# tschnz/Live-Video-Magnification

Measured on AMD Instinct MI355X. Metric: magnified frames/sec at 1080p, Laplace-motion 6 levels; % HBM roofline, higher is better.
Workload: dtype f32

## Files before the change

include/lvm_hip.h:

```cpp
#ifndef LVM_HIP_H
#define LVM_HIP_H
#include <stddef.h>
#include <stdint.h>
#ifdef __cplusplus
extern "C" {
#endif

enum lvm_mode { LVM_MODE_LAPLACE = 0, LVM_MODE_PHASE = 1, LVM_MODE_COLOR = 2, LVM_MODE_NONE = 3 };

enum lvm_status {
    LVM_OK = 0,
    LVM_ERR_INVALID = -1,
    LVM_ERR_HIP = -2,
    LVM_ERR_NO_DEVICE = -3,
    LVM_ERR_OOM = -4
};

typedef struct lvm_params {
    int32_t  mode;
    int32_t  levels;
    double   amplification;
    double   coWavelength;
    double   coLow;
    double   coHigh;
// ... 131 lines not shown
                       ptrdiff_t* chroma_stride);
int  lvm_canvas_convert_device(lvm_ctx* ctx, int fmt, const uint8_t* d_bgr, int w, int h, ptrdiff_t bgr_stride, ptrdiff_t bgr_frame_stride, int n_frames,
                               uint8_t* d_out, ptrdiff_t out_stride, ptrdiff_t out_frame_stride, void* hip_stream);

int  lvm_set_pipeline(lvm_ctx* ctx, int depth);
int  lvm_flush(lvm_ctx* ctx, void* hip_stream);

int  lvm_synchronize(lvm_ctx* ctx);

const char* lvm_last_error(lvm_ctx* ctx);

int  lvm_max_levels(int w, int h);
int  lvm_optimal_buffer_size(int fps);
void lvm_butterworth2(double Wn, double a[3], double b[3]);

int  lvm_debug_keep_float(lvm_ctx* ctx, int on);
int  lvm_debug_read_float(lvm_ctx* ctx, float* dst, size_t count);
int  lvm_debug_exact_lab(lvm_ctx* ctx, int on);
int  lvm_debug_clock_probe_start(lvm_ctx* ctx, double max_seconds);
int  lvm_debug_clock_probe_stop(lvm_ctx* ctx, double* mhz, double* seconds);
int  lvm_debug_sweep_u8_steps(lvm_ctx* ctx, uint32_t first_bits, uint64_t count, uint64_t* mismatches, uint32_t* first_bad_bits);
int  lvm_debug_lab_analytic(lvm_ctx* ctx, int on);
int  lvm_debug_trig_eval(lvm_ctx* ctx, int fn, const float* d_x, float* d_y, size_t n, void* stream);
#define LVM_LAB_LUT_ENTRIES (33 * 33 * 33 * 3)
int  lvm_get_lab_lut(lvm_ctx* ctx, int16_t* dst);
int  lvm_set_lab_lut(lvm_ctx* ctx, const int16_t* src);
int  lvm_profile_enable(lvm_ctx* ctx, int on);
int  lvm_profile_collect(lvm_ctx* ctx);
int  lvm_profile_only(lvm_ctx* ctx, const char* name);
int  lvm_profile_entry(lvm_ctx* ctx, int idx, char* name, size_t name_cap, double* total_ms,
                       long long* launches);
int  lvm_profile_variants(lvm_ctx* ctx, int idx, char* variants, size_t cap);
double lvm_algorithmic_bytes(int mode, int w, int h, int channels, int levels, double framerate);

#ifdef __cplusplus
}
#endif
#endif
```

live-video-magnification_amd/binding.py:

```python
import ctypes as C
import dataclasses
import enum
import os
import struct

import numpy as np

_HERE = os.path.dirname(os.path.abspath(__file__))
LIB_PATH = os.environ.get("LVM_HIP_LIB") or os.path.join(_HERE, "liblvm_hip.so")


class MagnificationMode(enum.IntEnum):
    Laplace = 0
    Phase = 1
    Color = 2
    None_ = 3


@dataclasses.dataclass
class MagnificationParams:
    mode: int = MagnificationMode.Laplace
    amplification: float = 0.0
    coWavelength: float = 0.0
    coLow: float = 0.0
# ... 43 lines not shown


class LvmOverlayLabel(C.Structure):
    _fields_ = [("x", C.c_int32), ("y", C.c_int32), ("w", C.c_int32), ("h", C.c_int32), ("n_classes", C.c_int32),
                ("cls", C.c_void_p), ("fn", C.c_void_p)]


class LvmPreprocessParams(C.Structure):
    _fields_ = [("downscale", C.c_int32), ("roi_enabled", C.c_int32), ("roiX", C.c_float), ("roiY", C.c_float),
                ("roiW", C.c_float), ("roiH", C.c_float), ("grayscale", C.c_int32)]


def to_c_preprocess(pre, grayscale=False):
    return LvmPreprocessParams(int(pre.downscale), 1 if pre.roiEnabled else 0, pre.roiX, pre.roiY, pre.roiW, pre.roiH,
                               1 if grayscale else 0)


class LvmError(RuntimeError):
    pass


SYMBOLS = ["lvm_create", "lvm_destroy", "lvm_reset", "lvm_process", "lvm_process_device", "lvm_process_device_frames", "lvm_set_pipeline", "lvm_flush", "lvm_synchronize",
           "lvm_last_error", "lvm_max_levels", "lvm_optimal_buffer_size", "lvm_butterworth2",
           "lvm_debug_keep_float", "lvm_debug_read_float", "lvm_debug_exact_lab", "lvm_debug_sweep_u8_steps", "lvm_debug_clock_probe_start", "lvm_debug_clock_probe_stop", "lvm_debug_lab_analytic", "lvm_debug_trig_eval", "lvm_get_lab_lut", "lvm_set_lab_lut", "lvm_profile_enable", "lvm_profile_collect", "lvm_profile_only",
           "lvm_profile_entry", "lvm_profile_variants", "lvm_algorithmic_bytes", "lvm_export_geometry", "lvm_export_frames", "lvm_export_set_overlay", "lvm_overlay_device", "lvm_tile_riesz_stage1", "lvm_tile_riesz_planes", "lvm_tile_riesz_stage2",
           "lvm_preprocess_geometry", "lvm_preprocess_device", "lvm_chain_process", "lvm_chain_process_batch",
           "lvm_set_max_frames", "lvm_host_alloc", "lvm_host_free", "lvm_compose_geometry", "lvm_compose_device", "lvm_chain_process_batch_ex",
           "lvm_chain_present", "lvm_mjpeg_bound", "lvm_mjpeg_encode_device", "lvm_export_frames_mjpeg", "lvm_mjpeg_decode_device", "lvm_export_mjpeg_frames", "lvm_mjpeg_set_restart_interval", "lvm_mjpeg_set_decoder", "lvm_mjpeg_set_samplings",
           "lvm_set_opencv_build", "lvm_get_opencv_build", "lvm_set_phase_on_gray", "lvm_get_phase_on_gray",
           "lvm_set_source_format", "lvm_get_source_format",
           "lvm_set_canvas_format", "lvm_get_canvas_format", "lvm_canvas_layout", "lvm_canvas_convert_device"]


def bind(lib):
    vp = C.c_void_p
    lib.lvm_create.argtypes = [C.c_int, C.c_int, C.POINTER(vp)]
    lib.lvm_destroy.argtypes = [vp]
    lib.lvm_destroy.restype = None
    lib.lvm_reset.argtypes = [vp]
    lib.lvm_process.argtypes = [vp, C.POINTER(LvmParams), vp, C.c_int, C.c_int, C.c_int, C.c_ssize_t,
                                vp, C.c_ssize_t, C.POINTER(C.c_int)]
    lib.lvm_process_device.argtypes = [vp, C.POINTER(LvmParams), vp, C.c_int, C.c_int, C.c_int, C.c_ssize_t,
                                       C.c_ssize_t, vp, C.c_ssize_t, C.c_ssize_t, C.POINTER(C.c_int), vp]
    lib.lvm_synchronize.argtypes = [vp]
    lib.lvm_process_device_frames.argtypes = [vp, C.POINTER(LvmParams), C.c_int, vp, C.c_int, C.c_int, C.c_int, C.c_ssize_t,
                                              C.c_ssize_t, C.c_ssize_t, vp, C.c_ssize_t, C.c_ssize_t, C.c_ssize_t,
                                              C.POINTER(C.c_int), vp]
    lib.lvm_set_pipeline.argtypes = [vp, C.c_int]
    lib.lvm_flush.argtypes = [vp, vp]
    lib.lvm_last_error.argtypes = [vp]
    lib.lvm_last_error.restype = C.c_char_p
    lib.lvm_max_levels.argtypes = [C.c_int, C.c_int]
    lib.lvm_optimal_buffer_size.argtypes = [C.c_int]
    lib.lvm_butterworth2.argtypes = [C.c_double, C.POINTER(C.c_double), C.POINTER(C.c_double)]
    lib.lvm_butterworth2.restype = None
    lib.lvm_debug_keep_float.argtypes = [vp, C.c_int]
    lib.lvm_debug_read_float.argtypes = [vp, vp, C.c_size_t]
    lib.lvm_debug_exact_lab.argtypes = [vp, C.c_int]
    lib.lvm_debug_lab_analytic.argtypes = [vp, C.c_int]
    lib.lvm_debug_clock_probe_start.argtypes = [vp, C.c_double]
    lib.lvm_debug_clock_probe_stop.argtypes = [vp, C.POINTER(C.c_double), C.POINTER(C.c_double)]
    lib.lvm_debug_sweep_u8_steps.argtypes = [vp, C.c_uint32, C.c_uint64, C.POINTER(C.c_uint64), C.POINTER(C.c_uint32)]
    lib.lvm_debug_trig_eval.argtypes = [vp, C.c_int, vp, vp, C.c_size_t, vp]
    lib.lvm_get_lab_lut.argtypes = [vp, vp]
    lib.lvm_set_lab_lut.argtypes = [vp, vp]
    lib.lvm_profile_enable.argtypes = [vp, C.c_int]
    lib.lvm_profile_collect.argtypes = [vp]
    lib.lvm_profile_only.argtypes = [vp, C.c_char_p]
    lib.lvm_profile_entry.argtypes = [vp, C.c_int, C.c_char_p, C.c_size_t, C.POINTER(C.c_double),
                                      C.POINTER(C.c_longlong)]
    lib.lvm_profile_variants.argtypes = [vp, C.c_int, C.c_char_p, C.c_size_t]
    lib.lvm_algorithmic_bytes.argtypes = [C.c_int, C.c_int, C.c_int, C.c_int, C.c_int, C.c_double]
    lib.lvm_algorithmic_bytes.restype = C.c_double
    ip = C.POINTER(C.c_int)
    lib.lvm_preprocess_geometry.argtypes = [C.POINTER(LvmPreprocessParams), C.c_int, C.c_int, C.c_int, ip, ip, ip, ip, ip, ip, ip]
    lib.lvm_preprocess_device.argtypes = [vp, C.POINTER(LvmPreprocessParams), vp, C.c_int, C.c_int, C.c_int, C.c_ssize_t,
                                          C.c_ssize_t, vp, C.c_ssize_t, C.c_ssize_t, vp]
    lib.lvm_chain_process.argtypes = [vp, C.POINTER(LvmPreprocessParams), C.POINTER(LvmParams), vp, C.c_int, C.c_int, C.c_int,
                                      C.c_ssize_t, vp, C.c_ssize_t, ip]
    lib.lvm_chain_process_batch.argtypes = [vp, C.POINTER(LvmPreprocessParams), C.POINTER(LvmParams), C.POINTER(vp), C.c_int, C.c_int,
                                            C.c_int, C.c_ssize_t, C.POINTER(vp), C.c_ssize_t, ip]
    lib.lvm_chain_process_batch_ex.argtypes = [vp, C.POINTER(LvmPreprocessParams), C.POINTER(LvmParams), C.POINTER(vp), C.c_int, C.c_int,
                                               C.c_int, C.c_ssize_t, C.POINTER(vp), C.c_ssize_t, C.POINTER(vp), C.c_ssize_t, ip]
    lib.lvm_chain_present.argtypes = [vp, C.POINTER(LvmPreprocessParams), C.POINTER(LvmParams), vp, C.c_int, C.c_int, C.c_int, C.c_ssize_t,
                                      vp, C.c_ssize_t, vp, C.c_ssize_t, ip]
    lib.lvm_export_geometry.argtypes = [C.POINTER(LvmPreprocessParams), C.c_int, C.c_int, C.c_int, C.c_int, ip, ip]
# ... 378 lines not shown

    def exact_lab(self, on=True):
        self._check(self.lib.lvm_debug_exact_lab(self.h, int(on)))

    def clock_probe_start(self, max_seconds=2.0):
        self._check(self.lib.lvm_debug_clock_probe_start(self.h, float(max_seconds)))

    def clock_probe_stop(self):
        mhz, sec = C.c_double(0), C.c_double(0)
        self._check(self.lib.lvm_debug_clock_probe_stop(self.h, C.byref(mhz), C.byref(sec)))
        return float(mhz.value), float(sec.value)

    def sweep_u8_steps(self, first_bits=0, count=1 << 32):
        bad, fb = C.c_uint64(0), C.c_uint32(0)
        self._check(self.lib.lvm_debug_sweep_u8_steps(self.h, first_bits, count, C.byref(bad), C.byref(fb)))
        return int(bad.value), int(fb.value)

    def lab_analytic(self, on=True):
        self._check(self.lib.lvm_debug_lab_analytic(self.h, int(on)))

    def trig_eval(self, fn, d_x, d_y, n, stream=None):
        self._check(self.lib.lvm_debug_trig_eval(self.h, int(fn), d_x, d_y, int(n), stream))

    def lab_lut(self):
        a = np.empty(LAB_LUT_ENTRIES, np.int16)
        self._check(self.lib.lvm_get_lab_lut(self.h, a.ctypes.data))
        return a

    def set_lab_lut(self, table):
        a = np.ascontiguousarray(table, np.int16).reshape(-1)
        assert a.size == LAB_LUT_ENTRIES
        self._check(self.lib.lvm_set_lab_lut(self.h, a.ctypes.data))

    def profile(self, on=True):
        self._check(self.lib.lvm_profile_enable(self.h, int(on)))

    def profile_only(self, name=None):
        self._check(self.lib.lvm_profile_only(self.h, name.encode() if name else None))

    def profile_collect(self):
        n = self.lib.lvm_profile_collect(self.h)
        out = {}
        for i in range(max(n, 0)):
            name = C.create_string_buffer(64)
            ms = C.c_double()
            cnt = C.c_longlong()
# ... 49 lines not shown
```

live-video-magnification_amd/csrc/color.hip:

```cpp
#include <cmath>
#include <cstdlib>

#include <vector>

#include "pyramid.h"

namespace lvm {

__device__ __forceinline__ int fkey(float f) { const int b = __float_as_int(f); return b >= 0 ? b : b ^ 0x7fffffff; }
__device__ __forceinline__ float fkey_inv(int k) { return __int_as_float(k >= 0 ? k : k ^ 0x7fffffff); }

constexpr int kMMCells = 32;
struct MinMax { int mn1[kMMCells], mx1[kMMCells], mn2[kMMCells], mx2[kMMCells]; };
__device__ __forceinline__ float mm_min(const int* cells) { int k = cells[0]; for (int i = 1; i < kMMCells; ++i) k = cells[i] < k ? cells[i] : k; return fkey_inv(k); }
__device__ __forceinline__ float mm_max(const int* cells) { int k = cells[0]; for (int i = 1; i < kMMCells; ++i) k = cells[i] > k ? cells[i] : k; return fkey_inv(k); }

__device__ __forceinline__ void block_minmax(float mn, float mx, int* gmn, int* gmx) {
    __shared__ float s_mn[256], s_mx[256];
    const int t = threadIdx.x;
    s_mn[t] = mn; s_mx[t] = mx;
    __syncthreads();
    for (int s = 128; s > 0; s >>= 1) {
        if (t < s) {
            s_mn[t] = s_mn[t + s] < s_mn[t] ? s_mn[t + s] : s_mn[t];
// ... 1073 lines not shown
    float* col1 = nullptr;
    int rows = 0, rows_ps = 0;
    float* win = nullptr; float* Y = nullptr; int cap = 0;
    int n = 0, slot0 = 0;
    int max_images = 0;
    bool yofs_strict = false;
    bool co_rows_ok = false;
    bool thin_dft = true;
    bool norm_in_up = true;
    float amp = 0.f;
    bool thin8_dft = true;
    long out_min_tasks = 2048;
    long out_min_tasks_lean = 900;
    bool up_rows = true;
    bool d0_rows_on = true;
    bool d01_on = true;
    int d01_rows_forced = 0;
    long d0_min_tasks = 4096;
    int out_rows = 16;
    int out_rows_lean = 36;
    bool out_lean = true;
    int thin_min_frames = 1;
    long rows_min_elems = 1 << 20;
    double* tw = nullptr; int tw_n = 0;
    double* tw_all = nullptr; int tw_all_max = 0; std::vector<size_t> tw_off;
    double* tw_own = nullptr; size_t tw_own_cap = 0;
    double* tw_stage[2] = {}; hipEvent_t tw_ev[2] = {}; int tw_turn = 0;
    bool long_dft = true;
    int long_from = kDftMaxN + 1;
    MinMax* mm = nullptr;
    int *xofs = nullptr, *yofs = nullptr; float *xa = nullptr, *ya = nullptr; YSlot* yslot = nullptr;
    int tcap = 0; float* tarena = nullptr; float* Gt[kMaxLevels + 1] = {}; float* upt[kMaxLevels + 1] = {}; float* col1t = nullptr; MinMax* mmt = nullptr;
    ~ColorState() override {
        void* p[] = {arena, win, Y, tw_all, tw_own, mm, xofs, yofs, yslot, xa, ya, tarena, mmt};
        for (void* q : p) if (q) (void)hipFree(q);
        for (int k = 0; k < 2; ++k) { if (tw_stage[k]) (void)hipHostFree(tw_stage[k]); if (tw_ev[k]) (void)hipEventDestroy(tw_ev[k]); }
    }
    int process(Ctx* c, const lvm_params& p, const FrameIO& io, hipStream_t s, int* produced) override;
    int batch_frames(const Ctx* c, const lvm_params& p, const FrameIO& io, int left) const override;
    int process_frames(Ctx* c, const lvm_params& p, const FrameIO& io, int nt, hipStream_t s) override;
};
constexpr int kColorBatchMax = 32;

static void color_layout(const ColorState* st, int nt, float** G, float** up, float** col1, ArenaCursor& a) {
    const int levels = st->levels;
    const size_t nL = st->g[levels].n;
// ... 95 lines not shown
    int l = 1;
    if (d01) {
        D01Args q;
        q.in = io.d_in; q.in_stride = (long)io.in_stride; q.in_sstride = (long)io.in_sstride; q.w = w; q.h = h;
        q.G2 = B.G[2]; q.w2 = st->g[2].w; q.h2 = st->g[2].h; q.h1 = st->g[1].h;
        q.strips_x = (st->g[2].w + D01_OUT - 1) / D01_OUT; q.rows = d01_rows; q.strips_y = (st->g[2].h + d01_rows - 1) / d01_rows;
        q.ntasks = (int)d01_tasks;
        LVM_LAUNCH(c, "col_down01", k_down01_rows<1>, dim3((unsigned)((d01_tasks + D01_THREADS / 64 - 1) / (D01_THREADS / 64))), dim3(D01_THREADS), s, q);
        l = 2;
    } else if (vec4 && st->d0_rows_on && d0_tasks > 0) {
        const dim3 gridr((unsigned)((d0_tasks + D0R_THREADS / 64 - 1) / (D0R_THREADS / 64)));
        LVM_LAUNCH_V(c, "col_down0", "strips", (k_down0_rows<false, FL_LUT_EXACT>), gridr, dim3(D0R_THREADS), s, io.d_in, (long)io.in_stride, (long)io.in_sstride,
                   w, h, B.G[1], g1.w, g1.h, c->lab, d0_sx, (g1.h + d0_rows - 1) / d0_rows, (int)d0_tasks, d0_rows, LabPlanes{nullptr, nullptr});
    } else if (vec4) {
        auto kv = k_down0_v4<false, FL_LUT_EXACT>;
        LVM_LAUNCH_V(c, "col_down0", "vec4", kv, grid0, blk, s, io.d_in, (long)io.in_stride, (long)io.in_sstride, w, h, B.G[1], g1.w, g1.h, c->lab, LabPlanes{nullptr, nullptr});
    } else {
        auto kd0 = (C == 3) ? k_down0<3, false, FL_LUT_EXACT> : k_down0<1, false, FL_LUT_EXACT>;
        LVM_LAUNCH_V(c, "col_down0", "bytes", kd0, grid0, blk, s, io.d_in, (long)io.in_stride, (long)io.in_sstride, w, h, B.G[1], g1.w, g1.h, c->lab, 1.0f, LabPlanes{nullptr, nullptr});
    }
    while (l < levels) {
        if (st->g[l].w % 4 == 0 && (long)st->g[l].n * planes >= st->rows_min_elems) {
            const LevelGeom &a = st->g[l], &b = st->g[l + 1];
            const int sx = (b.w + 127) / 128;
            int rows = 16;
            while (rows > 4 && (long)sx * ((b.h + rows - 1) / rows) * planes < 8192) rows >>= 1;
            const int sy = (b.h + rows - 1) / rows;
            const long ntasks = (long)sx * sy * planes;
            const dim3 grid((unsigned)((ntasks + PD_THREADS / 64 - 1) / (PD_THREADS / 64)));
            LVM_LAUNCH(c, LName("pyr_down_rows", l), k_pyr_down_rows<1>, grid, dim3(PD_THREADS), s, (const float*)B.G[l], a.w, a.h, B.G[l + 1], b.w, b.h,
                       sx, sy, (int)ntasks, rows);
            l += 1;
        } else if (levels - l >= 2) {
            const LevelGeom &a = st->g[l], &b1 = st->g[l + 1], &b2 = st->g[l + 2];
            const dim3 grid((b2.w + ML_T - 1) / ML_T, (b2.h + ML_T - 1) / ML_T, planes);
            LVM_LAUNCH(c, LName("pyr_down2", l), k_pyr_down_multi<2>, grid, blk, s, (const float*)B.G[l], a.w, a.h, B.G[l + 1], b1.w, b1.h, B.G[l + 2],
                       b2.w, b2.h, (float*)nullptr, 0, 0);
            l += 2;
        } else {
            const LevelGeom &a = st->g[l], &b = st->g[l + 1];
            const dim3 grid((b.w + 31) / 32, (b.h + 15) / 16, planes);
            LVM_LAUNCH(c, LName("pyr_down", l), k_pyr_down<1>, grid, blk, s, (const float*)B.G[l], a.w, a.h, B.G[l + 1], b.w, b.h);
            l += 1;
        }
    }
}

static int col_dft_kind(const ColorState* st, int n) {
    if (n < st->long_from && n <= kDftMaxN) return 0;
    return st->long_dft && n >= st->long_from && n <= kLongMaxN ? 1 : 2;
}

static int col_filter(Ctx* c, ColorState* st, const lvm_params& p, const ColBufs& B, int slot, int slot0, int n, hipStream_t s) {
    const int C = st->channels, NS = c->nstreams, levels = st->levels;
// ... 115 lines not shown
        LVM_LAUNCH_V(c, "col_out", "vec4", k_col_out_v4<true>, grid, blk, s, a);
    } else {
        auto k1 = (C == 3) ? k_col_out<3, false> : k_col_out<1, false>;
        auto k2 = (C == 3) ? k_col_out<3, true> : k_col_out<1, true>;
        LVM_LAUNCH_V(c, "col_minmax", "bytes", k1, grid, blk, s, a);
        LVM_LAUNCH_V(c, "col_out", "bytes", k2, grid, blk, s, a);
    }
}

static void color_switches(ColorState* st) {
    env_switch("LVM_COL_THIN_DFT", st->thin_dft);
    env_switch("LVM_COL_THIN8_DFT", st->thin8_dft);
    env_switch("LVM_COL_NORM_IN_UP", st->norm_in_up);
    env_switch("LVM_COL_UP_ROWS", st->up_rows);
    env_switch("LVM_D0_ROWS", st->d0_rows_on);
    env_switch("LVM_D0_MIN_TASKS", st->d0_min_tasks);
    if (env_switch("LVM_COL_OUT_ROWS", st->out_rows)) st->out_rows_lean = st->out_rows;
    env_switch("LVM_COL_OUT_LEAN", st->out_lean);
    env_switch("LVM_COL_DOWN01", st->d01_on);
    env_switch("LVM_COL_DOWN01_ROWS", st->d01_rows_forced);
    if (env_switch("LVM_COL_OUT_MIN_TASKS", st->out_min_tasks)) st->out_min_tasks_lean = st->out_min_tasks;
    env_switch("LVM_COL_THIN_MIN_FRAMES", st->thin_min_frames, [](int v) { return v >= 1; });
    env_switch("LVM_ROWS_MIN_ELEMS", st->rows_min_elems);
    env_switch("LVM_COL_LONG_DFT", st->long_dft);
    env_switch("LVM_COL_LONG_FROM", st->long_from, [](int x) { return x >= 2; });
}

int color_create(Ctx* c, int levels, const FrameIO& io, hipStream_t s) {
    ColorState* st = new ColorState();
    c->state = st;
    color_switches(st);
    int rc = color_alloc(c, st, io.w, io.h, io.channels, levels);
    if (rc == LVM_OK && c->max_frames > 1) rc = color_reserve_frames(c, st, c->max_frames, s);
    return rc;
}

int ColorState::process(Ctx* c, const lvm_params& p, const FrameIO& io, hipStream_t s, int* produced) {
    ColorState* st = this;
    *produced = 0;
    const ColBufs B{st->G, st->up, st->col1, st->mm, 1};
    col_down(c, st, io, B, s);
    const int maxImages = optimal_buffer_size((int)p.framerate);
    st->max_images = maxImages;
    {
        const int want = maxImages > 0 && maxImages <= 4096 ? maxImages + kColorBatchMax + 1 : 0;
        const int rc = color_reserve(c, st, st->n + 1 > want ? st->n + 1 : want, s);
// ... 101 lines not shown
```

live-video-magnification_amd/csrc/laplace.hip:

```cpp
#include <cstdlib>
#include <cstring>
#include <vector>

#include "pyramid.h"

namespace lvm {

struct UpArgs {
    const float* Gl;
    const float* Gn;
    const float* curn;
    float* hi; float* lo;
    float* cur;
    int w, h, wn, hn;
    float aHi, bHi, aLo, bLo, gain;
    int nt;
    long fsl, fsn;
};

template <bool SEED, int D>
__global__ __launch_bounds__(256) void k_lap_up(UpArgs a) {
    __shared__ float s_g[US_H][US_W + 1], s_c[US_H][US_W + 1];
    __shared__ float h_g[US_H][UT_W + 1], h_c[US_H][UT_W + 1];
    const Bid3 bq = xcd_swizzle3();
// ... 801 lines not shown
    struct Pending { bool valid = false; FrameIO io{}; lvm_params p{}; int par = 0; } pending;
    int par = 0, depth = 0;
    int tcap = 0; float* tarena = nullptr;
    float* Gt[kMaxLevels + 1] = {}; float* curt[kMaxLevels + 1] = {};
    uint16_t* iLp[2] = {}; uint32_t* iabp[2] = {};
    uint16_t* iLt = nullptr; uint32_t* iabt = nullptr;
    int split_min_nt = 1;
    long fin_min_tasks = 4096;
    long rows_min_elems = 2000000;
    int split_from = 3;
    int split_levels = 1;
    int up_rows = 1;
    long up_rows_max_blocks = 1024;
    bool d0_rows_on = true;
    bool d0_fused = true;
    int d0_fused_rows = 0;
    long d0_fused_groups = 0;
    long d0_fused_waves = 0;
    long d0_min_tasks = 4096;
    long fin_groups = 0;
    int fin_rows = 8;
    int up_depth_big = 1;
    int up_depth = 8;
    int pd_rows = 16;
    int fuse_down = 2;
    int tailT = 0;
    TailArgs tail{};
    ~LaplaceState() override {
        if (arena) (void)hipFree(arena);
        if (tarena) (void)hipFree(tarena);
    }
    int process(Ctx* c, const lvm_params& p, const FrameIO& io, hipStream_t s, int* produced) override;
    int batch_frames(const Ctx* c, const lvm_params&, const FrameIO&, int left) const override { return seeded && c->pipeline_depth == 0 ? left : 0; }
    int process_frames(Ctx* c, const lvm_params& p, const FrameIO& io, int nt, hipStream_t s) override;
    int flush(Ctx* c, hipStream_t s) override;
};

static void laplace_tail_plan(LaplaceState* st);
static int laplace_reserve_frames(Ctx* c, LaplaceState* st, int nt, hipStream_t s);

static void laplace_layout(LaplaceState* st, int NS, ArenaCursor& a) {
    const int levels = st->levels;
    for (int q = 0; q < 2; ++q)
        for (int l = 1; l <= levels; ++l) st->Gp[q][l] = a.take(st->g[l].n * st->planes);
    for (int l = 1; l <= levels; ++l) st->G[l] = st->Gp[0][l];
    const size_t npx = st->g[0].n * NS;
    if (st->planes == 3 * NS)
// ... 117 lines not shown
        auto kdl = fl == FL_LUT_EXACT ? k_down0_lut_rows<FL_LUT_EXACT> : k_down0_lut_rows<FL_LUT_FAST>;
        LVM_LAUNCH(c, "lap_down0_lut", kdl, dim3((unsigned)lap_d0l_groups(c, st)), dim3(D0L_THREADS), s, da);
    } else if (lap_vec4(io) && st->d0_rows_on && d0_tasks > 0) {
        auto kd0 = LVM_FL_PICK(fl, k_down0_rows, true);
        const dim3 gridr((unsigned)((d0_tasks + D0R_THREADS / 64 - 1) / (D0R_THREADS / 64)));
        LVM_LAUNCH_V(c, "lap_down0", "strips", kd0, gridr, dim3(D0R_THREADS), s, io.d_in, (long)io.in_stride, (long)io.in_sstride, io.w, io.h,
                   G[1], g1.w, g1.h, c->lab, d0_sx, (g1.h + d0_rows - 1) / d0_rows, (int)d0_tasks, d0_rows, lp);
    } else if (lap_vec4(io)) {
        auto kd0 = LVM_FL_PICK(fl, k_down0_v4, true);
        LVM_LAUNCH_V(c, "lap_down0", "vec4", kd0, grid0, blk, s, io.d_in, (long)io.in_stride, (long)io.in_sstride, io.w, io.h,
                   G[1], g1.w, g1.h, c->lab, lp);
    } else {
        auto kd0 = (C == 3) ? LVM_FL_PICK(fl, k_down0, 3, true) : k_down0<1, false, FL_LUT_EXACT>;
        LVM_LAUNCH_V(c, "lap_down0", "bytes", kd0, grid0, blk, s, io.d_in, (long)io.in_stride, (long)io.in_sstride, io.w, io.h,
                   G[1], g1.w, g1.h, c->lab, c->lab.a255, lp);
    }
    const bool use_tail = st->tailT && B.nt == 1 && !B.no_tail && !lap_split_now(st, B, first);
    const int down_end = use_tail ? st->tailT : levels;
    int l = 1;
    while (l < down_end) {
        const int left = down_end - l;
        if (st->g[l].w % 4 == 0 && (long)st->g[l].n * planes >= (l == 1 ? st->rows_min_elems / 2 : st->rows_min_elems)) {
            const LevelGeom &a = st->g[l], &b = st->g[l + 1];
            const int sx = (b.w + 127) / 128;
            int rows = st->pd_rows;
            while (rows > 4 && (long)sx * ((b.h + rows - 1) / rows) * planes < 8192) rows >>= 1;
            const int sy = (b.h + rows - 1) / rows;
            const long ntasks = (long)sx * sy * planes;
            const dim3 grid((unsigned)((ntasks + PD_THREADS / 64 - 1) / (PD_THREADS / 64)));
            LVM_LAUNCH(c, LName("pyr_down_rows", l), k_pyr_down_rows<0>, grid, dim3(PD_THREADS), s, (const float*)G[l], a.w, a.h, G[l + 1], b.w, b.h,
                       sx, sy, (int)ntasks, rows);
            l += 1;
        } else if (left >= 3 && st->fuse_down >= 3) {
            const LevelGeom &a = st->g[l], &b1 = st->g[l + 1], &b2 = st->g[l + 2], &b3 = st->g[l + 3];
            const dim3 grid((b3.w + ML_T - 1) / ML_T, (b3.h + ML_T - 1) / ML_T, planes);
            LVM_LAUNCH(c, LName("pyr_down3", l), k_pyr_down_multi<3>, grid, blk, s, (const float*)G[l], a.w, a.h, G[l + 1], b1.w, b1.h,
                       G[l + 2], b2.w, b2.h, G[l + 3], b3.w, b3.h);
            l += 3;
        } else if (left >= 2 && st->fuse_down >= 2) {
            const LevelGeom &a = st->g[l], &b1 = st->g[l + 1], &b2 = st->g[l + 2];
            const dim3 grid((b2.w + ML_T - 1) / ML_T, (b2.h + ML_T - 1) / ML_T, planes);
            LVM_LAUNCH(c, LName("pyr_down2", l), k_pyr_down_multi<2>, grid, blk, s, (const float*)G[l], a.w, a.h, G[l + 1], b1.w, b1.h,
                       G[l + 2], b2.w, b2.h, (float*)nullptr, 0, 0);
            l += 2;
        } else {
            const LevelGeom &a = st->g[l], &b = st->g[l + 1];
            const dim3 grid((b.w + DT_W - 1) / DT_W, (b.h + DT_H - 1) / DT_H, planes);
            LVM_LAUNCH(c, LName("pyr_down", l), k_pyr_down<0>, grid, blk, s, (const float*)G[l], a.w, a.h, G[l + 1], b.w, b.h);
            l += 1;
        }
    }
    if (use_tail) {
        float gains[kMaxLevels + 2];
        laplace_gains(io.w, io.h, levels, p.amplification, p.coWavelength, gains);
// ... 221 lines not shown
        lap_stage_a(c, st, p, io, lap_bufs_frame(st, 0), first, s);
        st->par = 1;
    } else {
        const int par = st->par;
        if (st->pending.valid) {
            LVM_HIP_TRY(c, hipEventRecord(c->ev_fork, s));
            LVM_HIP_TRY(c, hipStreamWaitEvent(c->aux_stream, c->ev_fork, 0));
            lap_stage_b(c, st, p, io, lap_bufs_frame(st, par), false, c->aux_stream);
            LVM_HIP_TRY(c, hipEventRecord(c->ev_join, c->aux_stream));
            lap_stage_a(c, st, st->pending.p, st->pending.io, lap_bufs_frame(st, st->pending.par), false, s);
            LVM_HIP_TRY(c, hipStreamWaitEvent(s, c->ev_join, 0));
        } else {
            lap_stage_b(c, st, p, io, lap_bufs_frame(st, par), false, s);
        }
        st->pending.valid = true; st->pending.io = io; st->pending.p = p; st->pending.par = par;
        st->par = par ^ 1;
    }
    LVM_HIP_TRY(c, hipGetLastError());
    st->seeded = true;
    *produced = 1;
    return LVM_OK;
}

}
```

live-video-magnification_amd/csrc/lvm_api.hip:

```cpp
#include <cmath>
#include <cstdio>
#include <cstdlib>
#include <cstring>
#include <new>

#include "lvm_internal.h"

struct lvm_ctx : lvm::Ctx {};

namespace lvm {

void prof_begin(Ctx* c, const char* name, hipStream_t s) {
    c->prof_skip = !c->prof_only.empty() && c->prof_only != name;
    if (c->prof_skip) return;
    int id = -1;
    for (size_t i = 0; i < c->prof_totals.size(); ++i)
        if (c->prof_totals[i].name == name) { id = (int)i; break; }
    if (id < 0) { ProfTotal t; t.name = name; c->prof_totals.push_back(t); id = (int)c->prof_totals.size() - 1; }
    ProfEvent e; e.name = id;
    (void)hipEventCreate(&e.e0); (void)hipEventCreate(&e.e1);
    (void)hipEventRecord(e.e0, s);
    c->prof_events.push_back(e);
}
void prof_variant(Ctx* c, const char* variant) {
// ... 1001 lines not shown
    LVM_HIP_TRY(c, hipSetDevice(c->device));
    return lvm::clock_probe_start(c, max_seconds);
}

int lvm_debug_clock_probe_stop(lvm_ctx* c, double* mhz, double* seconds) {
    if (!c) return LVM_ERR_INVALID;
    LVM_HIP_TRY(c, hipSetDevice(c->device));
    return lvm::clock_probe_stop(c, mhz, seconds);
}

int lvm_debug_lab_analytic(lvm_ctx* c, int on) { if (!c) return LVM_ERR_INVALID; c->lab_analytic = on != 0; return LVM_OK; }

int lvm_debug_trig_eval(lvm_ctx* c, int fn, const float* d_x, float* d_y, size_t n, void* hip_stream) {
    if (!c || fn < 0 || fn > 2 || (n && (!d_x || !d_y))) return LVM_ERR_INVALID;
    LVM_HIP_TRY(c, hipSetDevice(c->device));
    hipStream_t s = hip_stream ? (hipStream_t)hip_stream : c->own_stream;
    int rc = lvm::order_after_previous(c, s);
    if (rc != LVM_OK) return rc;
    rc = lvm::riesz_trig_eval(c, fn, d_x, d_y, n, s);
    lvm::mark_enqueued(c, s);
    return rc;
}

int lvm_get_lab_lut(lvm_ctx* c, int16_t* dst) {
    if (!c || !dst) return LVM_ERR_INVALID;
    std::memcpy(dst, c->lab_lut_compact.data(), c->lab_lut_compact.size() * sizeof(int16_t));
    return LVM_OK;
}

int lvm_set_lab_lut(lvm_ctx* c, const int16_t* src) {
    if (!c || !src) return LVM_ERR_INVALID;
    (void)hipSetDevice(c->device);
    for (size_t i = 0; i < (size_t)LVM_LAB_LUT_ENTRIES; ++i)
        if (src[i] < 0 || src[i] > 16384) { c->err = "lvm_set_lab_lut: entry outside [0, 16384]"; return LVM_ERR_INVALID; }
    lvm::sync_streams(c);
    c->lab_lut_compact.assign(src, src + LVM_LAB_LUT_ENTRIES);
    ++c->lab_lut_gen;
    return lvm::upload_lab_lut(c);
}

int lvm_debug_read_float(lvm_ctx* c, float* dst, size_t count) {
    if (!c || !dst) return LVM_ERR_INVALID;
    if (!c->d_float.p || count > c->float_count) { c->err = "no float frame kept"; return LVM_ERR_INVALID; }
    lvm::sync_streams(c);
    LVM_HIP_TRY(c, hipMemcpy(dst, c->d_float.p, count * sizeof(float), hipMemcpyDeviceToHost));
    return LVM_OK;
// ... 94 lines not shown
```

live-video-magnification_amd/csrc/lvm_internal.h:

```cpp
#pragma once
#include <hip/hip_runtime.h>

#include <cstddef>
#include <cstdint>
#include <cstring>
#include <cstdio>
#include <cstdlib>
#include <string>
#include <utility>
#include <vector>

#include "lvm_hip.h"
#include "lab_lut.h"
#include <lvm_gfx950.h>

namespace lvm {

constexpr int kMaxLevels = 24;

__device__ __forceinline__ int reflect101(int p, int len) {
    if (len == 1) return 0;
    while (p < 0 || p >= len) p = (p < 0) ? -p : 2 * len - 2 - p;
    return p;
}
// ... 374 lines not shown
    ModeState* state = nullptr;
    DevBuf d_in, d_out;
    bool keep_float = false;
    DevBuf d_float; size_t float_count = 0;
    bool profiling = false;
    std::string prof_only; bool prof_skip = false;
    std::vector<ProfEvent> prof_events;
    std::vector<ProfTotal> prof_totals;
    int pipeline_depth = 0;
    hipStream_t aux_stream = nullptr;
    hipEvent_t ev_fork = nullptr, ev_join = nullptr;
    std::vector<std::pair<hipStream_t, hipEvent_t>> caller_events;
    bool caller_overflow = false;
    hipStream_t last_stream = nullptr;
    hipEvent_t ev_last = nullptr, ev_own = nullptr, ev_spill = nullptr;
    bool last_marked = false;
    int max_frames = 0;
    bool exact_lab = false;
    bool lab_analytic = false;
    uint32_t* d_lab_ab = nullptr; uint4* d_lab_Lcells = nullptr;
    LabLut lab_lut{};
    int num_cus = 256;
    const void* fin_occ_kernel = nullptr; int fin_occ_groups = 0;
    std::vector<int16_t> lab_lut_compact;
    void* pre_tables = nullptr;
    DevBuf d_pre_in, d_pre_out, d_chain_out;
    DevBuf d_canvas;
    DevBuf d_pre_tap;
    hipStream_t up_stream = nullptr, down_stream = nullptr;
    std::vector<hipEvent_t> ev_up, ev_done;
    void* mjpeg = nullptr;
    void* mjpeg_dec = nullptr;
    int mjpeg_decoder = LVM_MJPEG_DECODER_REPLICATE;
    unsigned mjpeg_samplings = LVM_MJPEG_SAMPLING_420;
    unsigned opencv_build = 0;
    bool phase_on_gray = false;
    int source_format = LVM_PIX_BGR;
    int canvas_format = LVM_PIX_BGR;
    DevBuf d_canvas_yuv;
    unsigned lab_lut_gen = 0;
};

inline int lab_flavour(const Ctx* c) { return c->lab_analytic ? FL_ANALYTIC : (c->exact_lab ? FL_LUT_EXACT : FL_LUT_FAST); }
#define LVM_FL_PICK(fl, K, ...) ((fl) == FL_ANALYTIC ? K<__VA_ARGS__, FL_ANALYTIC> : ((fl) == FL_LUT_EXACT ? K<__VA_ARGS__, FL_LUT_EXACT> : K<__VA_ARGS__, FL_LUT_FAST>))
#define LVM_FL_PICK0(fl, K) ((fl) == FL_ANALYTIC ? K<FL_ANALYTIC> : ((fl) == FL_LUT_EXACT ? K<FL_LUT_EXACT> : K<FL_LUT_FAST>))

// ... 118 lines not shown
int mjpeg_decode_device(Ctx* c, const uint8_t* jpegs, const size_t* offsets, int n, int w, int h, uint8_t* d_bgr, ptrdiff_t stride, ptrdiff_t fstride, hipStream_t s);
int mjpeg_drain(Ctx* c, uint8_t* out_host, size_t upto_call);
void mjpeg_abort(Ctx* c);
int mjpeg_finish(Ctx* c, size_t total_frames, uint8_t* out_host, size_t* offsets, hipStream_t s);
int overlay_set(Ctx* c, int n, const lvm_overlay_label* labels);
int overlay_device(Ctx* c, uint8_t* d_canvas, int cw, int chh, ptrdiff_t stride, ptrdiff_t fstride, int n_frames, hipStream_t s);
void overlay_release(Ctx* c);
struct CanvasLayout { size_t bytes, plane1, plane2; ptrdiff_t cstride; };
const char* canvas_layout(int fmt, int w, int h, ptrdiff_t stride, CanvasLayout* out);
int canvas_yuv_device(Ctx* c, int fmt, const uint8_t* d_bgr, int w, int h, ptrdiff_t bgr_stride, ptrdiff_t bgr_fstride, int n_frames, uint8_t* d_out,
                      ptrdiff_t out_stride, ptrdiff_t out_fstride, hipStream_t s, bool check_only = false);
int canvas_yuv_fused(Ctx* c, int fmt, int split, const uint8_t* d_orig, int ow, int oh, int och, ptrdiff_t ostride, const uint8_t* d_proc, int pw, int ph,
                     int pch, ptrdiff_t pstride, uint8_t* d_out, ptrdiff_t out_stride, hipStream_t s);
int compose_device(Ctx* c, int split, const uint8_t* d_orig, int ow, int oh, int och, ptrdiff_t ostride, ptrdiff_t osstride,
                   const uint8_t* d_proc, int pw, int ph, int pch, ptrdiff_t pstride, ptrdiff_t psstride, uint8_t* d_canvas,
                   ptrdiff_t cstride, ptrdiff_t csstride, hipStream_t s);

int laplace_create(Ctx* c, int levels, const FrameIO& io, hipStream_t s);
int riesz_create(Ctx* c, int levels, const FrameIO& io, hipStream_t s);
int color_create(Ctx* c, int levels, const FrameIO& io, hipStream_t s);
int riesz_tile_residual(Ctx* c, float* d_dst, int* rw, int* rh, hipStream_t s);
int riesz_tile_finish(Ctx* c, const lvm_params& p, const FrameIO& io, const float* d_residual, hipStream_t s);
int riesz_trig_eval(Ctx* c, int fn, const float* d_x, float* d_y, size_t n, hipStream_t s);

void build_lab_tables(float gamma_u8[256], float invgamma[4096], float fwd[9], float inv[9]);
int clock_probe_start(Ctx* c, double max_seconds);
int clock_probe_stop(Ctx* c, double* mhz, double* seconds);
int sweep_u8_steps(Ctx* c, unsigned long long first, unsigned long long count, unsigned long long* bad, unsigned long long* first_bad, hipStream_t s);
bool build_u8_steps(const float invgamma[4096], uint32_t steps[2 * kU8StepSlices]);
void build_lab_lut_compact(std::vector<int16_t>& compact);
void lab_lut_device_tables(const int16_t* compact, std::vector<uint32_t>& ab, std::vector<int16_t>& lcells);
bool lab_lut_fine_index_ok();
int upload_lab_lut(Ctx* c);
void butterworth2(double Wn, double a[3], double b[3]);
int optimal_buffer_size(int fps);

}
```

live-video-magnification_amd/csrc/pyramid.h:

```cpp
#pragma once
#include "lvm_internal.h"

namespace lvm {

constexpr int DT_W = 32, DT_H = 16;
constexpr int DS_W = 2 * DT_W + 3, DS_H = 2 * DT_H + 3;

template <int C>
__device__ __forceinline__ void pyrdown_tile(float (&s_src)[C][DS_H][DS_W], float (&s_row)[C][DS_H][DT_W],
                                             float* __restrict__ dst, int dw, int dh, size_t dplane,
                                             int ox0, int oy0) {
    const int tid = threadIdx.x;
    for (int i = tid; i < C * DS_H * DT_W; i += 256) {
        const int c = i / (DS_H * DT_W);
        const int r = i - c * (DS_H * DT_W);
        const int ly = r / DT_W, x = r - ly * DT_W;
        const float* s = &s_src[c][ly][2 * x];
        s_row[c][ly][x] = s[2] * 6.f + (s[1] + s[3]) * 4.f + s[0] + s[4];
    }
    __syncthreads();
    for (int i = tid; i < C * DT_H * DT_W; i += 256) {
        const int c = i / (DT_H * DT_W);
        const int r = i - c * (DT_H * DT_W);
        const int y = r / DT_W, x = r - y * DT_W;
// ... 525 lines not shown
        const int r4 = rv;
        l1(nA0, nA1, t4);
#pragma unroll
        for (int c = 0; c < 3; ++c) {
            float e3 = t3[c], e4 = t4[c];
            if (r3 >= h1) { const int k = 2 * h1 - 2 - r3 - (2 * Y - 2); e3 = k == 0 ? w0[c] : (k == 1 ? w1[c] : w2r[c]); }
            if (r4 >= h1) { const int k = 2 * h1 - 2 - r4 - (2 * Y - 2); e4 = k == 0 ? w0[c] : (k == 1 ? w1[c] : (k == 2 ? w2r[c] : e3)); }
            w3[c] = e3; w4[c] = e4;
        }
        if (top && Y == 0) {
#pragma unroll
            for (int c = 0; c < 3; ++c) { w0[c] = w4[c]; w1[c] = w3[c]; }
        }
        if (owner) {
#pragma unroll
            for (int c = 0; c < 3; ++c)
                dst[c * plane + (size_t)Y * w2] = __builtin_fmaf(w2r[c], 6.f, __builtin_fmaf(w1[c] + w3[c], 4.f, w0[c] + w4[c])) * (1.f / 256.f);
        }
#pragma unroll
        for (int c = 0; c < 3; ++c) { w0[c] = w2r[c]; w1[c] = w3[c]; w2r[c] = w4[c]; }
    }
}

constexpr int PD_THREADS = 256;
template <int TU>
__global__ __launch_bounds__(PD_THREADS) void k_pyr_down_rows(const float* __restrict__ src, int w, int h,
                                                              float* __restrict__ dst, int dw, int dh,
                                                              int strips_x, int strips_y, int ntasks, int rows) {
    const int wave = __builtin_amdgcn_readfirstlane((int)(threadIdx.x >> 6)), lane = threadIdx.x & 63;
    const int task = blockIdx.x * (PD_THREADS / 64) + wave;
    if (task >= ntasks) return;
    const int pl = task / (strips_x * strips_y);
    const int r = task - pl * (strips_x * strips_y);
    const int ty = r / strips_x, tx = r - ty * strips_x;
    const int ox = tx * 128 + 2 * lane, oy0 = ty * rows;
    if (ox >= dw) return;
    const float* sp = src + (size_t)pl * ((size_t)w * h);
    float* dp = dst + (size_t)pl * ((size_t)dw * dh);
    const int c = 2 * ox;
    const bool interior = c >= 2 && c + 4 < w;
    unsigned off[7];
#pragma unroll
    for (int k = 0; k < 7; ++k) off[k] = 4u * (unsigned)reflect101(c - 2 + k, w);
    const unsigned offc = 4u * (unsigned)c;
    auto hpair = [&](int sy, float& ha, float& hb) __attribute__((always_inline)) {
        const char* row = reinterpret_cast<const char*>(sp + (size_t)reflect101(sy, h) * w);
        float t[7];
        if (interior) {
            const float2 a = *reinterpret_cast<const float2*>(row + offc - 8);
            const float4 m = *reinterpret_cast<const float4*>(row + offc);
            t[0] = a.x; t[1] = a.y; t[2] = m.x; t[3] = m.y; t[4] = m.z; t[5] = m.w;
            t[6] = *reinterpret_cast<const float*>(row + offc + 16);
        } else {
#pragma unroll
            for (int k = 0; k < 7; ++k) t[k] = *reinterpret_cast<const float*>(row + off[k]);
        }
        ha = t[2] * 6.f + (t[1] + t[3]) * 4.f + t[0] + t[4];
        hb = t[4] * 6.f + (t[3] + t[5]) * 4.f + t[2] + t[6];
    };
    const int yend = oy0 + rows < dh ? oy0 + rows : dh;
    float a0, a1, a2, a3, a4, b0, b1, b2, b3, b4;
    hpair(2 * oy0 - 2, a0, b0); hpair(2 * oy0 - 1, a1, b1); hpair(2 * oy0, a2, b2);
    const bool pair_store = (dw & 1) == 0;
    for (int oy = oy0; oy < yend; ++oy) {
        hpair(2 * oy + 1, a3, b3); hpair(2 * oy + 2, a4, b4);
        const float va = (a2 * 6.f + (a1 + a3) * 4.f + a0 + a4) * (1.f / 256.f);
        const float vb = (b2 * 6.f + (b1 + b3) * 4.f + b0 + b4) * (1.f / 256.f);
        float* q = dp + (size_t)oy * dw + ox;
        if (pair_store) *reinterpret_cast<float2*>(q) = make_float2(va, vb);
        else { q[0] = va; if (ox + 1 < dw) q[1] = vb; }
        a0 = a2; a1 = a3; a2 = a4; b0 = b2; b1 = b3; b2 = b4;
    }
}

constexpr int ML_T = 8;
template <int NL>
__global__ __launch_bounds__(256) void k_pyr_down_multi(const float* __restrict__ src, int w0, int h0,
                                                        float* __restrict__ d1, int w1, int h1,
                                                        float* __restrict__ d2, int w2, int h2,
                                                        float* __restrict__ d3, int w3, int h3) {
    constexpr int T3 = ML_T, T2 = (NL == 3) ? 2 * ML_T : ML_T, T1 = 2 * T2;
    constexpr int R2 = (NL == 3) ? 2 * T3 + 3 : T2;
    constexpr int R1 = 2 * R2 + 3;
    constexpr int R0 = 2 * R1 + 3;
    __shared__ float s0[R0][R0 + 1];
    __shared__ float ht[R0][R1 + 1];
    __shared__ float s1[R1][R1 + 1];
    __shared__ float s2[R2][R2 + 1];
    const int tid = threadIdx.x;
    const size_t pl = blockIdx.z;
    const float* sp = src + pl * ((size_t)w0 * h0);
    const int o2x = (NL == 3) ? 2 * (blockIdx.x * T3) - 2 : blockIdx.x * T2, o2y = (NL == 3) ? 2 * (blockIdx.y * T3) - 2 : blockIdx.y * T2;
    const int o1x = 2 * o2x - 2, o1y = 2 * o2y - 2;
    const int o0x = 2 * o1x - 2, o0y = 2 * o1y - 2;
    for (int i = tid; i < R0 * R0; i += 256) {
// ... 94 lines not shown
```

Measured before the change: 51440.

## Share pyramid-down horizontal taps via DPP and pick strip rows by occupancy model

The row-strip pyramid-down kernel now has each lane load a single aligned float4 per source row and get neighbour taps from adjacent lanes through DPP shifts, with edge lanes acting as halo. Previously each lane issued overlapping float2/float4/float loads. Each wave now writes 124 output columns instead of 128. Rows per strip are chosen by a cost model built on queried occupancy (resident waves) instead of a fixed halve-until-8192-tasks rule. The aim is fewer redundant loads and better balance across CUs, at the cost of two idle halo lanes per wave and a cost heuristic that may be wrong for some shapes.

```diff
diff --git a/include/lvm_hip.h b/include/lvm_hip.h
--- a/include/lvm_hip.h
+++ b/include/lvm_hip.h
@@ -177,6 +177,7 @@
 int  lvm_debug_sweep_u8_steps(lvm_ctx* ctx, uint32_t first_bits, uint64_t count, uint64_t* mismatches, uint32_t* first_bad_bits);
 int  lvm_debug_lab_analytic(lvm_ctx* ctx, int on);
 int  lvm_debug_trig_eval(lvm_ctx* ctx, int fn, const float* d_x, float* d_y, size_t n, void* stream);
+long lvm_debug_pd_rows(lvm_ctx* ctx, int dw, int dh, long planes, long resident, int forced, int* rows);
 #define LVM_LAB_LUT_ENTRIES (33 * 33 * 33 * 3)
 int  lvm_get_lab_lut(lvm_ctx* ctx, int16_t* dst);
 int  lvm_set_lab_lut(lvm_ctx* ctx, const int16_t* src);
diff --git a/live-video-magnification_amd/binding.py b/live-video-magnification_amd/binding.py
--- a/live-video-magnification_amd/binding.py
+++ b/live-video-magnification_amd/binding.py
@@ -89,7 +89,7 @@
 
 SYMBOLS = ["lvm_create", "lvm_destroy", "lvm_reset", "lvm_process", "lvm_process_device", "lvm_process_device_frames", "lvm_set_pipeline", "lvm_flush", "lvm_synchronize",
            "lvm_last_error", "lvm_max_levels", "lvm_optimal_buffer_size", "lvm_butterworth2",
-           "lvm_debug_keep_float", "lvm_debug_read_float", "lvm_debug_exact_lab", "lvm_debug_sweep_u8_steps", "lvm_debug_clock_probe_start", "lvm_debug_clock_probe_stop", "lvm_debug_lab_analytic", "lvm_debug_trig_eval", "lvm_get_lab_lut", "lvm_set_lab_lut", "lvm_profile_enable", "lvm_profile_collect", "lvm_profile_only",
+           "lvm_debug_keep_float", "lvm_debug_read_float", "lvm_debug_exact_lab", "lvm_debug_sweep_u8_steps", "lvm_debug_clock_probe_start", "lvm_debug_clock_probe_stop", "lvm_debug_lab_analytic", "lvm_debug_trig_eval", "lvm_debug_pd_rows", "lvm_get_lab_lut", "lvm_set_lab_lut", "lvm_profile_enable", "lvm_profile_collect", "lvm_profile_only",
            "lvm_profile_entry", "lvm_profile_variants", "lvm_algorithmic_bytes", "lvm_export_geometry", "lvm_export_frames", "lvm_export_set_overlay", "lvm_overlay_device", "lvm_tile_riesz_stage1", "lvm_tile_riesz_planes", "lvm_tile_riesz_stage2",
            "lvm_preprocess_geometry", "lvm_preprocess_device", "lvm_chain_process", "lvm_chain_process_batch",
            "lvm_set_max_frames", "lvm_host_alloc", "lvm_host_free", "lvm_compose_geometry", "lvm_compose_device", "lvm_chain_process_batch_ex",
@@ -129,6 +129,8 @@
     lib.lvm_debug_clock_probe_stop.argtypes = [vp, C.POINTER(C.c_double), C.POINTER(C.c_double)]
     lib.lvm_debug_sweep_u8_steps.argtypes = [vp, C.c_uint32, C.c_uint64, C.POINTER(C.c_uint64), C.POINTER(C.c_uint32)]
     lib.lvm_debug_trig_eval.argtypes = [vp, C.c_int, vp, vp, C.c_size_t, vp]
+    lib.lvm_debug_pd_rows.argtypes = [vp, C.c_int, C.c_int, C.c_long, C.c_long, C.c_int, C.POINTER(C.c_int)]
+    lib.lvm_debug_pd_rows.restype = C.c_long
     lib.lvm_get_lab_lut.argtypes = [vp, vp]
     lib.lvm_set_lab_lut.argtypes = [vp, vp]
     lib.lvm_profile_enable.argtypes = [vp, C.c_int]
@@ -553,6 +555,13 @@
     def trig_eval(self, fn, d_x, d_y, n, stream=None):
         self._check(self.lib.lvm_debug_trig_eval(self.h, int(fn), d_x, d_y, int(n), stream))
 
+    def pd_rows(self, dw, dh, planes, forced=0):
+        rows = C.c_int(0)
+        n = self.lib.lvm_debug_pd_rows(self.h, int(dw), int(dh), int(planes), 0, int(forced), C.byref(rows))
+        if n < 0:
+            self._check(int(n))
+        return int(rows.value), int(n)
+
     def lab_lut(self):
         a = np.empty(LAB_LUT_ENTRIES, np.int16)
         self._check(self.lib.lvm_get_lab_lut(self.h, a.ctypes.data))
diff --git a/live-video-magnification_amd/csrc/color.hip b/live-video-magnification_amd/csrc/color.hip
--- a/live-video-magnification_amd/csrc/color.hip
+++ b/live-video-magnification_amd/csrc/color.hip
@@ -1119,6 +1119,7 @@
     bool out_lean = true;
     int thin_min_frames = 1;
     long rows_min_elems = 1 << 20;
+    int pd_rows = 0;
     double* tw = nullptr; int tw_n = 0;
     double* tw_all = nullptr; int tw_all_max = 0; std::vector<size_t> tw_off;
     double* tw_own = nullptr; size_t tw_own_cap = 0;
@@ -1260,14 +1261,10 @@
     while (l < levels) {
         if (st->g[l].w % 4 == 0 && (long)st->g[l].n * planes >= st->rows_min_elems) {
             const LevelGeom &a = st->g[l], &b = st->g[l + 1];
-            const int sx = (b.w + 127) / 128;
-            int rows = 16;
-            while (rows > 4 && (long)sx * ((b.h + rows - 1) / rows) * planes < 8192) rows >>= 1;
-            const int sy = (b.h + rows - 1) / rows;
-            const long ntasks = (long)sx * sy * planes;
-            const dim3 grid((unsigned)((ntasks + PD_THREADS / 64 - 1) / (PD_THREADS / 64)));
+            const PdRowsGeom q = pyr_down_rows_geom<1>(c, b.w, b.h, planes, st->pd_rows);
+            const dim3 grid((unsigned)((q.ntasks + PD_THREADS / 64 - 1) / (PD_THREADS / 64)));
             LVM_LAUNCH(c, LName("pyr_down_rows", l), k_pyr_down_rows<1>, grid, dim3(PD_THREADS), s, (const float*)B.G[l], a.w, a.h, B.G[l + 1], b.w, b.h,
-                       sx, sy, (int)ntasks, rows);
+                       q.sx, q.sy, (int)q.ntasks, q.rows);
             l += 1;
         } else if (levels - l >= 2) {
             const LevelGeom &a = st->g[l], &b1 = st->g[l + 1], &b2 = st->g[l + 2];
@@ -1429,6 +1426,7 @@
     if (env_switch("LVM_COL_OUT_MIN_TASKS", st->out_min_tasks)) st->out_min_tasks_lean = st->out_min_tasks;
     env_switch("LVM_COL_THIN_MIN_FRAMES", st->thin_min_frames, [](int v) { return v >= 1; });
     env_switch("LVM_ROWS_MIN_ELEMS", st->rows_min_elems);
+    env_switch("LVM_PD_ROWS", st->pd_rows, [](int v) { return v >= 1; });
     env_switch("LVM_COL_LONG_DFT", st->long_dft);
     env_switch("LVM_COL_LONG_FROM", st->long_from, [](int x) { return x >= 2; });
 }
diff --git a/live-video-magnification_amd/csrc/laplace.hip b/live-video-magnification_amd/csrc/laplace.hip
--- a/live-video-magnification_amd/csrc/laplace.hip
+++ b/live-video-magnification_amd/csrc/laplace.hip
@@ -847,7 +847,7 @@
     int fin_rows = 8;
     int up_depth_big = 1;
     int up_depth = 8;
-    int pd_rows = 16;
+    int pd_rows = 0;
     int fuse_down = 2;
     int tailT = 0;
     TailArgs tail{};
@@ -1011,14 +1011,10 @@
         const int left = down_end - l;
         if (st->g[l].w % 4 == 0 && (long)st->g[l].n * planes >= (l == 1 ? st->rows_min_elems / 2 : st->rows_min_elems)) {
             const LevelGeom &a = st->g[l], &b = st->g[l + 1];
-            const int sx = (b.w + 127) / 128;
-            int rows = st->pd_rows;
-            while (rows > 4 && (long)sx * ((b.h + rows - 1) / rows) * planes < 8192) rows >>= 1;
-            const int sy = (b.h + rows - 1) / rows;
-            const long ntasks = (long)sx * sy * planes;
-            const dim3 grid((unsigned)((ntasks + PD_THREADS / 64 - 1) / (PD_THREADS / 64)));
+            const PdRowsGeom q = pyr_down_rows_geom<0>(c, b.w, b.h, planes, st->pd_rows);
+            const dim3 grid((unsigned)((q.ntasks + PD_THREADS / 64 - 1) / (PD_THREADS / 64)));
             LVM_LAUNCH(c, LName("pyr_down_rows", l), k_pyr_down_rows<0>, grid, dim3(PD_THREADS), s, (const float*)G[l], a.w, a.h, G[l + 1], b.w, b.h,
-                       sx, sy, (int)ntasks, rows);
+                       q.sx, q.sy, (int)q.ntasks, q.rows);
             l += 1;
         } else if (left >= 3 && st->fuse_down >= 3) {
             const LevelGeom &a = st->g[l], &b1 = st->g[l + 1], &b2 = st->g[l + 2], &b3 = st->g[l + 3];
@@ -1286,4 +1282,10 @@
     return LVM_OK;
 }
 
-}
+long laplace_pd_rows(Ctx* c, int dw, int dh, long planes, long resident, int forced, int* rows) {
+    long tasks = 0;
+    *rows = pyr_down_rows_choice(dw, dh, planes, resident > 0 ? resident : pyr_down_resident<0>(c), forced, &tasks);
+    return tasks;
+}
+
+}
diff --git a/live-video-magnification_amd/csrc/lvm_api.hip b/live-video-magnification_amd/csrc/lvm_api.hip
--- a/live-video-magnification_amd/csrc/lvm_api.hip
+++ b/live-video-magnification_amd/csrc/lvm_api.hip
@@ -1047,6 +1047,12 @@
     return rc;
 }
 
+long lvm_debug_pd_rows(lvm_ctx* c, int dw, int dh, long planes, long resident, int forced, int* rows) {
+    if (!rows || dw < 1 || dh < 1 || planes < 1 || forced < 0 || (!c && resident <= 0)) return LVM_ERR_INVALID;
+    if (c && resident <= 0) (void)hipSetDevice(c->device);
+    return lvm::laplace_pd_rows(c, dw, dh, planes, resident, forced, rows);
+}
+
 int lvm_get_lab_lut(lvm_ctx* c, int16_t* dst) {
     if (!c || !dst) return LVM_ERR_INVALID;
     std::memcpy(dst, c->lab_lut_compact.data(), c->lab_lut_compact.size() * sizeof(int16_t));
diff --git a/live-video-magnification_amd/csrc/lvm_internal.h b/live-video-magnification_amd/csrc/lvm_internal.h
--- a/live-video-magnification_amd/csrc/lvm_internal.h
+++ b/live-video-magnification_amd/csrc/lvm_internal.h
@@ -420,6 +420,7 @@
     LabLut lab_lut{};
     int num_cus = 256;
     const void* fin_occ_kernel = nullptr; int fin_occ_groups = 0;
+    long pd_occ_waves[2] = {};
     std::vector<int16_t> lab_lut_compact;
     void* pre_tables = nullptr;
     DevBuf d_pre_in, d_pre_out, d_chain_out;
@@ -584,6 +585,7 @@
 int riesz_tile_residual(Ctx* c, float* d_dst, int* rw, int* rh, hipStream_t s);
 int riesz_tile_finish(Ctx* c, const lvm_params& p, const FrameIO& io, const float* d_residual, hipStream_t s);
 int riesz_trig_eval(Ctx* c, int fn, const float* d_x, float* d_y, size_t n, hipStream_t s);
+long laplace_pd_rows(Ctx* c, int dw, int dh, long planes, long resident, int forced, int* rows);
 
 void build_lab_tables(float gamma_u8[256], float invgamma[4096], float fwd[9], float inv[9]);
 int clock_probe_start(Ctx* c, double max_seconds);
diff --git a/live-video-magnification_amd/csrc/pyramid.h b/live-video-magnification_amd/csrc/pyramid.h
--- a/live-video-magnification_amd/csrc/pyramid.h
+++ b/live-video-magnification_amd/csrc/pyramid.h
@@ -571,7 +571,40 @@
     }
 }
 
-constexpr int PD_THREADS = 256;
+#ifndef LVM_PD_DPP
+#define LVM_PD_DPP 1
+#endif
+#ifndef LVM_PD_PREFETCH
+#define LVM_PD_PREFETCH 0
+#endif
+#ifndef LVM_PD_MODEL
+#define LVM_PD_MODEL 1
+#endif
+constexpr int PD_THREADS = 256, PD_OUT = LVM_PD_DPP ? 124 : 128;
+
+inline int pyr_down_rows_choice(int dw, int dh, long planes, long resident, int forced, long* tasks_out) {
+    const long sx = (dw + PD_OUT - 1) / PD_OUT;
+    const auto tasks_of = [&](int r) { return sx * ((dh + r - 1) / r) * planes; };
+    int best = 4;
+    if (forced >= 1) best = forced;
+    else if (LVM_PD_MODEL) {
+        if (resident < 1) resident = 1;
+        long best_cost = -1, any_cost = -1; int any = 4;
+        for (int r = 4; r <= 48; ++r) {
+            const long tasks = tasks_of(r), cost = ((tasks + resident - 1) / resident) * (2 * r + 3);
+            if (any_cost < 0 || cost < any_cost) { any_cost = cost; any = r; }
+            if (tasks * 5 < resident * 3) continue;
+            if (best_cost < 0 || cost < best_cost) { best_cost = cost; best = r; }
+        }
+        if (best_cost < 0) best = any;
+    } else {
+        best = 16;
+        while (best > 4 && tasks_of(best) < 8192) best >>= 1;
+    }
+    *tasks_out = tasks_of(best);
+    return best;
+}
+
 template <int TU>
 __global__ __launch_bounds__(PD_THREADS) void k_pyr_down_rows(const float* __restrict__ src, int w, int h,
                                                               float* __restrict__ dst, int dw, int dh,
@@ -582,10 +615,47 @@
     const int pl = task / (strips_x * strips_y);
     const int r = task - pl * (strips_x * strips_y);
     const int ty = r / strips_x, tx = r - ty * strips_x;
-    const int ox = tx * 128 + 2 * lane, oy0 = ty * rows;
-    if (ox >= dw) return;
+    const int oy0 = ty * rows;
     const float* sp = src + (size_t)pl * ((size_t)w * h);
     float* dp = dst + (size_t)pl * ((size_t)dw * dh);
+    const int yend = oy0 + rows < dh ? oy0 + rows : dh;
+    float a0, a1, a2, a3, a4, b0, b1, b2, b3, b4;
+#if LVM_PD_DPP
+    const int ngroups = w >> 2;
+    const int g = tx * (PD_OUT / 2) - 1 + lane;
+    const bool left_mirror = g < 0, right_mirror = g >= ngroups;
+    const int gl = left_mirror ? 0 : (right_mirror ? ngroups - 1 : g);
+    const int ox = 2 * g;
+    const bool owner = lane >= 1 && lane <= 62 && g >= 0 && ox < dw;
+    auto fetch = [&](int sy) __attribute__((always_inline)) {
+        return *reinterpret_cast<const float4*>(sp + (size_t)reflect101(sy, h) * w + 4u * (unsigned)gl);
+    };
+    auto hrow = [&](const float4 p, float& ha, float& hb) __attribute__((always_inline)) {
+        const float give2 = p.z, give3 = left_mirror ? p.y : p.w, give0 = right_mirror ? p.z : p.x;
+        const float L2 = dpp_shr1(give2), L3 = dpp_shr1(give3), R0 = dpp_shl1(give0);
+        ha = p.x * 6.f + (L3 + p.y) * 4.f + L2 + p.z;
+        hb = p.z * 6.f + (p.y + p.w) * 4.f + p.x + R0;
+    };
+    hrow(fetch(2 * oy0 - 2), a0, b0); hrow(fetch(2 * oy0 - 1), a1, b1); hrow(fetch(2 * oy0), a2, b2);
+#if LVM_PD_PREFETCH
+    float4 n3 = fetch(2 * oy0 + 1), n4 = fetch(2 * oy0 + 2);
+#endif
+    for (int oy = oy0; oy < yend; ++oy) {
+#if LVM_PD_PREFETCH
+        const float4 c3 = n3, c4 = n4;
+        if (oy + 1 < yend) { n3 = fetch(2 * oy + 3); n4 = fetch(2 * oy + 4); }
+#else
+        const float4 c3 = fetch(2 * oy + 1), c4 = fetch(2 * oy + 2);
+#endif
+        hrow(c3, a3, b3); hrow(c4, a4, b4);
+        const float va = (a2 * 6.f + (a1 + a3) * 4.f + a0 + a4) * (1.f / 256.f);
+        const float vb = (b2 * 6.f + (b1 + b3) * 4.f + b0 + b4) * (1.f / 256.f);
+        if (owner) *reinterpret_cast<float2*>(dp + (size_t)oy * dw + ox) = make_float2(va, vb);
+        a0 = a2; a1 = a3; a2 = a4; b0 = b2; b1 = b3; b2 = b4;
+    }
+#else
+    const int ox = tx * 128 + 2 * lane;
+    if (ox >= dw) return;
     const int c = 2 * ox;
     const bool interior = c >= 2 && c + 4 < w;
     unsigned off[7];
@@ -607,8 +677,6 @@
         ha = t[2] * 6.f + (t[1] + t[3]) * 4.f + t[0] + t[4];
         hb = t[4] * 6.f + (t[3] + t[5]) * 4.f + t[2] + t[6];
     };
-    const int yend = oy0 + rows < dh ? oy0 + rows : dh;
-    float a0, a1, a2, a3, a4, b0, b1, b2, b3, b4;
     hpair(2 * oy0 - 2, a0, b0); hpair(2 * oy0 - 1, a1, b1); hpair(2 * oy0, a2, b2);
     const bool pair_store = (dw & 1) == 0;
     for (int oy = oy0; oy < yend; ++oy) {
@@ -620,6 +688,27 @@
         else { q[0] = va; if (ox + 1 < dw) q[1] = vb; }
         a0 = a2; a1 = a3; a2 = a4; b0 = b2; b1 = b3; b2 = b4;
     }
+#endif
+}
+template <int TU>
+inline long pyr_down_resident(Ctx* c) {
+    static_assert(TU == 0 || TU == 1, "one slot per instance");
+    if (c->pd_occ_waves[TU] <= 0) {
+        int n = 0;
+#ifdef __HIPCC__
+        if (hipOccupancyMaxActiveBlocksPerMultiprocessor(&n, k_pyr_down_rows<TU>, PD_THREADS, 0) != hipSuccess) { n = 0; (void)hipGetLastError(); }
+#endif
+        c->pd_occ_waves[TU] = (long)(n > 0 ? n : 8) * c->num_cus * (PD_THREADS / 64);
+    }
+    return c->pd_occ_waves[TU];
+}
+struct PdRowsGeom { int sx, sy, rows; long ntasks; };
+template <int TU>
+inline PdRowsGeom pyr_down_rows_geom(Ctx* c, int dw, int dh, long planes, int forced) {
+    PdRowsGeom q;
+    q.rows = pyr_down_rows_choice(dw, dh, planes, pyr_down_resident<TU>(c), forced, &q.ntasks);
+    q.sx = (dw + PD_OUT - 1) / PD_OUT; q.sy = (dh + q.rows - 1) / q.rows;
+    return q;
 }
 
 constexpr int ML_T = 8;
```

New measurement: 52360 (median of 6 runs). +1.8%, better.
